# wangty537/raft_optical_flow

Measured on AMD Instinct MI355X. Metric: image-pairs/s at Sintel 436x1024, 32 iters; corr-lookup GB/s vs HBM peak, higher is better.
Workload: dtype fp32 (convs: f16x3 split MFMA, fp32 accumulate); 1 GPU; RAFT-full inference, 436x1024 padded to 440x1024, 1 pair(s)/GPU/step, iters=32, all-pairs corr, hipGraph; global_batch=1, parallelism=frame-pair sharding x1

## Files before the change

include/raft_hip.h:

```cpp
#ifndef RAFT_HIP_H_
#define RAFT_HIP_H_

#include <stddef.h>

#ifdef __cplusplus
extern "C" {
#endif

#define RAFT_HIP_ABI_VERSION 19

#define RAFT_E_INVALID (-1)
#define RAFT_E_ALIGN (-2)

typedef void* raft_stream_t;

int raft_hip_abi_version(void);
const char* raft_hip_arch(void);
const char* raft_hip_last_error(void);
const char* raft_hip_source_hash(void);
int raft_debug_launch_span(int enable);
int raft_debug_launch_span_read(unsigned long long* host, int n);
int raft_debug_fill_lds_nan(raft_stream_t stream);

size_t raft_corr_pyramid_floats(int B, int H, int W, int num_levels);
int raft_corr_build(const float* fmap1, const float* fmap2, int ld, int B, int H, int W, int C,
                    int num_levels, float sqrt_c, float* pyramid, raft_stream_t stream);
int raft_corr_build_prec(const float* fmap1, const float* fmap2, int ld, int B, int H, int W, int C,
                         int num_levels, float sqrt_c, int precision, float* pyramid, raft_stream_t stream);
size_t raft_corr_build_ws_bytes(int B, int H, int W, int C);
size_t raft_corr_build_ws_bytes_prec(int B, int H, int W, int C, int precision);
int raft_corr_build_ws(const float* fmap1, const float* fmap2, int ld, int B, int H, int W, int C,
                       int num_levels, float sqrt_c, int precision, float* pyramid, void* ws, size_t ws_bytes,
                       raft_stream_t stream);
int raft_corr_pyramid_level(const float* pyramid, int B, int H, int W, int num_levels, int level,
                            float* out, raft_stream_t stream);

int raft_corr_lookup(const float* pyramid, int B, int H, int W, int num_levels, int radius,
                     const float* coords, int coords_layout, float* out, int out_ld, int out_layout,
                     float* flow_out, int flow_ld, int* range_flag, raft_stream_t stream);
int raft_corr_lookup_convf1(const float* pyramid, int B, int H, int W, int num_levels, int radius,
                            const float* coords, int coords_layout, float* out, int out_ld, int out_layout,
                            float* flow_out, int flow_ld, int* range_flag, const float* f1_weight,
                            const float* f1_bias, int f1_n, int f1_k, int f1_precision, float* f1_out,
                            int f1_out_ld, int* f1_range_flag, raft_stream_t stream);
int raft_convf1_flow(const float* coords, int coords_layout, int B, int H, int W, const float* f1_weight,
                     const float* f1_bias, int f1_n, int f1_k, int f1_precision, float* f1_out, int f1_out_ld,
                     int* f1_range_flag, raft_stream_t stream);

int raft_corr_lookup_conv(const float* pyramid, int B, int H, int W, int num_levels, int radius,
                          const float* coords, float* flow_out, int flow_ld, int* range_flag, int precision,
                          const void* c1_weight, const float* c1_bias, int c1_n, float* c1_out, int c1_out_ld,
                          int* c1_range_flag, const void* f1_weight, const float* f1_bias, int f1_n, int f1_k,
                          float* f1_out, int f1_out_ld, int* f1_range_flag, raft_stream_t stream);
size_t raft_lookup_conv_weight_floats(int n, int k_pad);
int raft_lookup_conv_pack_weight(const void* split_weight, int n_pad, int k_pad, int n, void* out,
                                 raft_stream_t stream);
// ... 249 lines not shown
```

raft_optical_flow_amd/_lib.py:

```python
from __future__ import annotations

import ctypes
import os
import threading

_HERE = os.path.dirname(os.path.abspath(__file__))
LIB_PATH = os.environ.get("RAFT_HIP_LIB") or os.path.join(_HERE, "libraft_hip.so")

c_int = ctypes.c_int
c_float = ctypes.c_float
c_size_t = ctypes.c_size_t
c_long = ctypes.c_long
c_void_p = ctypes.c_void_p
c_char_p = ctypes.c_char_p
P = c_void_p

RAFT_CONV_VEC = 0
RAFT_CONV_GATHER = 1

PREC_FP32 = 0
PREC_F16X3 = 1
PREC_F16 = 2
PREC_BF16 = 3
PRECISIONS = {"fp32": PREC_FP32, "f16x3": PREC_F16X3, "f16": PREC_F16, "bf16": PREC_BF16}
# ... 99 lines not shown
    f = ConvForm()
    call("raft_conv2d_form", ctypes.byref(p), ctypes.byref(f))
    return f


def conv_pair_form(p0: ConvParams, p1: ConvParams):
    f = (ConvForm * 2)()
    one = c_int(0)
    call("raft_conv2d_pair_form", ctypes.byref(p0), ctypes.byref(p1), f, ctypes.byref(one))
    return f[0], f[1], bool(one.value)


_PROTOS = {
    "raft_hip_abi_version": (c_int, []),
    "raft_hip_arch": (c_char_p, []),
    "raft_hip_last_error": (c_char_p, []),
    "raft_hip_source_hash": (c_char_p, []),
    "raft_debug_fill_lds_nan": (c_int, [P]),
    "raft_corr_pyramid_floats": (c_size_t, [c_int, c_int, c_int, c_int]),
    "raft_corr_build": (c_int, [P, P, c_int, c_int, c_int, c_int, c_int, c_int, c_float, P, P]),
    "raft_corr_build_prec": (c_int, [P, P, c_int, c_int, c_int, c_int, c_int, c_int, c_float, c_int, P, P]),
    "raft_corr_build_ws_bytes": (c_size_t, [c_int, c_int, c_int, c_int]),
    "raft_corr_build_ws_bytes_prec": (c_size_t, [c_int, c_int, c_int, c_int, c_int]),
    "raft_corr_build_ws": (c_int, [P, P, c_int, c_int, c_int, c_int, c_int, c_int, c_float, c_int, P, P, c_size_t, P]),
    "raft_corr_pyramid_level": (c_int, [P, c_int, c_int, c_int, c_int, c_int, P, P]),
    "raft_corr_lookup": (c_int, [P, c_int, c_int, c_int, c_int, c_int, P, c_int, P, c_int, c_int, P, c_int, P, P]),
    "raft_corr_lookup_convf1": (c_int, [P, c_int, c_int, c_int, c_int, c_int, P, c_int, P, c_int, c_int, P, c_int, P,
                                        P, P, c_int, c_int, c_int, P, c_int, P, P]),
    "raft_convf1_flow": (c_int, [P, c_int, c_int, c_int, c_int, P, P, c_int, c_int, c_int, P, c_int, P, P]),
    "raft_corr_lookup_conv": (c_int, [P, c_int, c_int, c_int, c_int, c_int, P, P, c_int, P, c_int, P, P, c_int, P,
                                      c_int, P, P, P, c_int, c_int, P, c_int, P, P]),
    "raft_lookup_conv_weight_floats": (c_size_t, [c_int, c_int]),
    "raft_lookup_conv_pack_weight": (c_int, [P, c_int, c_int, c_int, P, P]),
    "raft_alt_corr_forward": (c_int, [P, P, P, P, c_int, c_int, c_int, c_int, c_int, c_int, c_int, c_int, c_float, P]),
    "raft_alt_corr_forward_prec": (c_int, [P, P, P, P, c_int, c_int, c_int, c_int, c_int, c_int, c_int, c_int, c_float,
                                           c_int, P]),
    "raft_alt_corr_lookup_levels_prec": (c_int, [P, P, P, P, c_int, P, c_int, P, c_int, c_int, c_int, c_int, c_int,
                                                 c_int, ctypes.c_float, P, c_int, P, c_int, P]),
    "raft_alt_corr_lookup_nhwc_prec": (c_int, [P, P, P, c_int, c_float, P, c_int, c_int, c_int, c_int, c_int, c_int,
                                               c_int, c_int, c_float, P, c_int, P, c_int, P]),
    "raft_alt_corr_lookup_levels": (c_int, [P, P, P, P, c_int, P, c_int, P, c_int, c_int, c_int, c_int, c_int, c_int,
                                            ctypes.c_float, P, c_int, P, P]),
    "raft_alt_corr_lookup_nhwc": (c_int, [P, P, P, c_int, c_float, P, c_int, c_int, c_int, c_int, c_int, c_int, c_int,
                                          c_int, c_float, P, c_int, P, P]),
    "raft_alt_corr_backward": (c_int, [P, P, P, P, P, P, P, c_int, c_int, c_int, c_int, c_int, c_int, c_int, c_int,
                                       P, c_size_t, P]),
# ... 134 lines not shown
```

raft_optical_flow_amd/csrc/corr_pyramid.hip:

```cpp
#include "lookup_common.hpp"

namespace raft {
namespace {



constexpr int CB_BM = 64, CB_BN = 64, CB_BK = 32, CB_LDSK = CB_BK + 4;

struct CorrBuildArgs {
  const float* f1;
  const float* f2;
  int ld, H, W, C, P;
  float sqrt_c;
  float* pyr;
  Level l0, l1;
  int has_l1;
  int nbx;
  int nt;
  int B, mt, ntl, gm, nfast, xcd;
};

template <bool X3>
__global__ __launch_bounds__(256) void corr_build_kernel(CorrBuildArgs a) {
  constexpr int STAGE = (CB_BM + CB_BN) * CB_LDSK;
// ... 290 lines not shown
        const int xx = tj * 4 + c;
        float v = 0.f;
        if (by * 4 + yy < a.l1.h && bx * 8 + xx < a.l1.w) {
          const float* t = T + row * CB2_TLD + (2 * yy) * 16 + 2 * xx;
          const float2 u0 = *reinterpret_cast<const float2*>(t), u1 = *reinterpret_cast<const float2*>(t + 16);
          v = (((u0.x + u0.y) + u1.x) + u1.y) / 4.0f;
        }
        v4[c] = v;
      }
      f32x4* dst = reinterpret_cast<f32x4*>(a.pyr + a.l1.off + ((long)b * a.P + p1) * a.l1.mapsz +
                                            ((long)by * a.l1.tw + tx1) * 16 + e);
      if (a.nt)
        __builtin_nontemporal_store(v4, dst);
      else
        *dst = v4;
    }
  }
}

constexpr int CB4_T = 256;
constexpr int CB4_ROW = 64;
constexpr int CB4_STAGE = 2 * CB4_T * CB4_ROW;
constexpr int CB4_NS = 4;

struct CB4Args {
  const char* s1;
  const char* s2;
  unsigned sbytes;
  int H, W, P, nh;
  float sqrt_c;
  float* pyr;
  Level l0, l1, l2;
  int nt;
  int qt, ttx, tt;
  long units;
  f32x4* sink;
};

__global__ __launch_bounds__(256) void corr_split4_kernel(const float* __restrict__ f, int ld, long npix, int C,
                                                          char* __restrict__ out) {
  const long i = (long)blockIdx.x * 256 + threadIdx.x;
  const int ng = C / 4;
  if (i >= npix * ng) return;
  const long px = i / ng;
  const int g = (int)(i - px * ng);
  const f32x4 v = *reinterpret_cast<const f32x4*>(f + px * ld + 4 * g);
  h4 hi, lo;
#pragma unroll
  for (int e = 0; e < 4; ++e) {
    const _Float16 h = (_Float16)v[e];
    hi[e] = h;
    lo[e] = (_Float16)(v[e] - (float)h);
  }
  char* r = out + px * (long)C * 4 + (g >> 2) * CB4_ROW + (g & 3) * 8;
  *reinterpret_cast<h4*>(r) = hi;
  *reinterpret_cast<h4*>(r + 32) = lo;
}

#ifdef CB4_STAMPS
__device__ unsigned long long g_cb4stamp[8 * 8 * 1024];
__device__ __forceinline__ unsigned long long cb4_clock() {
  unsigned long long t;
  __builtin_amdgcn_sched_barrier(0);
// ... 18 lines not shown
  constexpr int TQ = NW == 8 ? CB4_T : CB4_T / 2;
  constexpr int ROWS = CB4_T + TQ;
  constexpr int NS = NW == 8 ? CB4_NS : 3;
  constexpr int AHEAD = NS - 1;
  constexpr int STAGE = ROWS * CB4_ROW;
  constexpr int NDMA = ROWS / 16 / NW;
  constexpr int TDMA = 16 / NW;
#ifdef CB4_STAMPS
  unsigned long long cb4_t[6] = {}, cb4_prev = cb4_clock();
  const unsigned long long cb4_start = cb4_prev;
  int cb4_units = 0;
#endif
  constexpr int NSTORE = 8 * (4 + (L1 ? 1 : 0)) + (L2 ? 4 : 0);
  __shared__ __attribute__((aligned(1024))) char smem[NS * STAGE];
  const int lane = threadIdx.x & 63;
  const int w = __builtin_amdgcn_readfirstlane(threadIdx.x >> 6);
  const int wm = w & 3, wn = NW == 8 ? w >> 2 : 0;
  const int m = lane & 31, h = lane >> 5;
  const long grid = gridDim.x;
  const unsigned rowb = (unsigned)a.nh * CB4_ROW;
  const __amdgpu_buffer_rsrc_t rq = make_rsrc(a.s1, a.sbytes), rt = make_rsrc(a.s2, a.sbytes);
  struct Unit {
    int b, q0, ty0, tx0;
  };
  auto unit_at = [&](long u) {
    Unit t;
    const long per = (long)a.qt * a.tt;
    t.b = (int)(u / per);
    const long r = u - (long)t.b * per;
    const int qi = (int)(r / a.tt), ti = (int)(r - (long)qi * a.tt);
    t.q0 = qi * TQ;
    t.ty0 = (ti / a.ttx) * 16;
    t.tx0 = (ti % a.ttx) * 16;
    return t;
  };
  unsigned voff[NDMA];
  auto set_offsets = [&](const Unit& t) {
#pragma unroll
    for (int k = 0; k < NDMA; ++k) {
      const int row = 16 * (w + NW * k) + (lane >> 2);
      const unsigned lq = (unsigned)((lane & 3) ^ ((row >> 1) & 3));
      bool ok;
      long px;
      if (k < TDMA) {
        const int R = row, mm = R & 31, c = (R >> 5) & 1;
        const int h2 = t.ty0 + 4 * (R >> 6) + (mm >> 3), w2 = t.tx0 + 8 * c + 4 * ((mm >> 2) & 1) + (mm & 3);
        ok = h2 < a.H && w2 < a.W;
        px = (long)t.b * a.P + (long)h2 * a.W + w2;
      } else {
        const int p1 = t.q0 + row - CB4_T;
        ok = p1 < a.P;
        px = (long)t.b * a.P + p1;
      }
      voff[k] = ok ? (unsigned)px * rowb + lq * 16u : OFF_INVALID;
    }
  };
  const long total = a.units;
  long u_is = blockIdx.x;
  int s_is = 0;
  long g_is = 0;
  if (u_is >= total) return;
  set_offsets(unit_at(u_is));
  auto issue = [&]() {
    const bool live = u_is < total;
    char* st = smem + (g_is % NS) * STAGE;
#pragma unroll
    for (int k = 0; k < NDMA; ++k)
      dma16(k < TDMA ? rt : rq, st + (w + NW * k) * 1024, live ? voff[k] : OFF_INVALID, (unsigned)s_is * CB4_ROW);
    ++g_is;
    if (++s_is == a.nh) {
      s_is = 0;
      u_is += grid;
      if (u_is < total) set_offsets(unit_at(u_is));
    }
  };
#pragma unroll
  for (int k = 0; k < AHEAD; ++k) issue();
  const int arow0 = wm * 64 + m, brow0 = CB4_T + wn * 128 + m;
  f32x16 acc[2][4];
#pragma unroll
  for (int c = 0; c < 2; ++c)
#pragma unroll
    for (int j = 0; j < 4; ++j) acc[c][j] = f32x16{};
  long g = 0;
  int since = AHEAD;
  for (long u = blockIdx.x; u < total; u += grid) {
    for (int s = 0; s < a.nh; ++s, ++g, ++since) {
      CB4_ST(5);
      if (since <= AHEAD - 1)
        wait_vm<NDMA * (AHEAD - 1) + NSTORE>();
      else
        wait_vm<NDMA * (AHEAD - 1)>();
      CB4_ST(0);
      asm volatile("s_barrier" ::: "memory");
      CB4_ST(1);
      issue();
      CB4_ST(2);
      const char* st = smem + (g % NS) * STAGE;
      h8 ah[2], al[2], bh[4], bl[4];
#pragma unroll
      for (int c = 0; c < 2; ++c) {
        const int row = arow0 + 32 * c, sw = (row >> 1) & 3;
        ah[c] = *reinterpret_cast<const h8*>(st + row * CB4_ROW + ((h ^ sw) << 4));
        al[c] = *reinterpret_cast<const h8*>(st + row * CB4_ROW + (((2 + h) ^ sw) << 4));
      }
#pragma unroll
      for (int j = 0; j < 4; ++j) {
        const int row = brow0 + 32 * j, sw = (row >> 1) & 3;
        bh[j] = *reinterpret_cast<const h8*>(st + row * CB4_ROW + ((h ^ sw) << 4));
        bl[j] = *reinterpret_cast<const h8*>(st + row * CB4_ROW + (((2 + h) ^ sw) << 4));
      }
#pragma unroll
      for (int c = 0; c < 2; ++c)
#pragma unroll
        for (int j = 0; j < 4; ++j) acc[c][j] = __builtin_amdgcn_mfma_f32_32x32x16_f16(ah[c], bh[j], acc[c][j], 0, 0, 0);
#pragma unroll
      for (int c = 0; c < 2; ++c)
#pragma unroll
        for (int j = 0; j < 4; ++j) acc[c][j] = __builtin_amdgcn_mfma_f32_32x32x16_f16(al[c], bh[j], acc[c][j], 0, 0, 0);
#pragma unroll
      for (int c = 0; c < 2; ++c)
#pragma unroll
        for (int j = 0; j < 4; ++j) acc[c][j] = __builtin_amdgcn_mfma_f32_32x32x16_f16(ah[c], bl[j], acc[c][j], 0, 0, 0);
      CB4_ST(3);
    }
    const Unit t = unit_at(u);
    const int ty = t.ty0 / 4 + wm;
#pragma unroll
    for (int j = 0; j < 4; ++j) {
      const int p1 = t.q0 + wn * 128 + j * 32 + m;
      const bool qok = p1 < a.P;
      const long qb = (long)t.b * a.P + (qok ? p1 : 0);
      float l2v[2];
#pragma unroll
      for (int c = 0; c < 2; ++c) {
        const int tx = t.tx0 / 4 + 2 * c + h;
        float v[16];
#pragma unroll
        for (int r = 0; r < 16; ++r) v[r] = acc[c][j][r] / a.sqrt_c;
        {
          float rt[4][4];
#pragma unroll
          for (int e = 0; e < 4; ++e) {
#pragma unroll
            for (int i = 0; i < 4; ++i) rt[e][i] = v[4 * i + e];
            quad_transpose(rt[e]);
          }
          const int qr = lane & 3;
#pragma unroll
          for (int i = 0; i < 4; ++i) {
            const int pi = t.q0 + wn * 128 + j * 32 + (m & ~3) + i;
            const bool ok = pi < a.P && ty < a.l0.th && tx < a.l0.tw;
            f32x4* dst = ok ? reinterpret_cast<f32x4*>(a.pyr + a.l0.off + ((long)t.b * a.P + pi) * a.l0.mapsz +
                                                       ((long)ty * a.l0.tw + tx) * 16) + qr
                            : a.sink + 4 * lane + i;
            const f32x4 x = {rt[0][i], rt[1][i], rt[2][i], rt[3][i]};
            if (a.nt)
              __builtin_nontemporal_store(x, dst);
            else
              *dst = x;
          }
        }
        if constexpr (L1) {
          float pv[2][2];
#pragma unroll
          for (int ya = 0; ya < 2; ++ya)
#pragma unroll
            for (int xb = 0; xb < 2; ++xb) {
              const float s = ((v[8 * ya + 2 * xb] + v[8 * ya + 2 * xb + 1]) + v[8 * ya + 4 + 2 * xb]) + v[8 * ya + 4 + 2 * xb + 1];
              const bool in = 2 * ty + ya < a.l1.h && 2 * tx + xb < a.l1.w;
              pv[ya][xb] = in ? s / 4.0f : 0.f;
            }
          const float o0 = __shfl_xor(pv[1 - h][0], 32), o1 = __shfl_xor(pv[1 - h][1], 32);
          const f32x4 row4 = h == 0 ? f32x4{pv[0][0], pv[0][1], o0, o1} : f32x4{o0, o1, pv[1][0], pv[1][1]};
// ... 6 lines not shown
            __builtin_nontemporal_store(row4, dst);
          else
            *dst = row4;
          if constexpr (L2) {
            const bool in2 = ty < a.l2.h && tx < a.l2.w;
            l2v[c] = in2 ? (((pv[0][0] + pv[0][1]) + pv[1][0]) + pv[1][1]) / 4.0f : 0.f;
          }
        }
      }
      if constexpr (L2) {
        const float o0 = __shfl_xor(l2v[0], 32), o1 = __shfl_xor(l2v[1], 32);
        const int ty2 = t.ty0 >> 4, tx2 = t.tx0 >> 4;
        const bool ok = qok && h == 0 && ty2 < a.l2.th && tx2 < a.l2.tw;
        f32x4* dst = ok ? reinterpret_cast<f32x4*>(a.pyr + a.l2.off + qb * a.l2.mapsz + ((long)ty2 * a.l2.tw + tx2) * 16 +
                                                   wm * 4)
                        : a.sink + 4 * lane;
        const f32x4 row4 = {l2v[0], o0, l2v[1], o1};
        if (a.nt)
          __builtin_nontemporal_store(row4, dst);
        else
          *dst = row4;
      }
    }
#pragma unroll
    for (int c = 0; c < 2; ++c)
#pragma unroll
      for (int j = 0; j < 4; ++j) acc[c][j] = f32x16{};
    since = 0;
    CB4_ST(4);
#ifdef CB4_STAMPS
    ++cb4_units;
#endif
  }
  wait_vm<0>();
#ifdef CB4_STAMPS
  if (lane == 0 && blockIdx.x < 1024) {
    unsigned long long* gs = g_cb4stamp + ((long)blockIdx.x * 8 + w) * 8;
    for (int k = 0; k < 6; ++k) gs[k] = cb4_t[k];
    gs[6] = cb4_clock() - cb4_start;
    gs[7] = (unsigned long long)cb4_units;
  }
#endif
}

__global__ void pool2_tiled_kernel(const float* pyr, float* out_base, long n_maps, Level src,
                                   Level dst) {
  const long total = n_maps * dst.mapsz;
  for (long i = blockIdx.x * (long)blockDim.x + threadIdx.x; i < total; i += (long)gridDim.x * blockDim.x) {
    const long q = i / dst.mapsz;
    const int r = (int)(i - q * dst.mapsz);
    const int tile = r >> 4, e = r & 15;
    const int y = (tile / dst.tw) * 4 + (e >> 2), x = (tile % dst.tw) * 4 + (e & 3);
    float v = 0.f;
    if (y < dst.h && x < dst.w) {
      const float* m = pyr + src.off + q * src.mapsz;
// ... 495 lines not shown
#ifdef CB4_STAMPS
extern "C" int raft_debug_cb4stamps(unsigned long long* host, int n) {
  return (int)hipMemcpyFromSymbol(host, HIP_SYMBOL(g_cb4stamp), sizeof(unsigned long long) * (size_t)n);
}
#endif

extern "C" size_t raft_corr_build_ws_bytes(int B, int H, int W, int C) {
  if (B <= 0 || H <= 0 || W <= 0 || C <= 0) return 0;
  return 2 * (size_t)B * H * W * C * 4 + 4096;
}

namespace raft {
static bool corr_build4_shape(int B, int H, int W, int C, int precision) {
  if (env_off("RAFT_CORR_BUILD4")) return false;
  return precision == RAFT_PREC_F16X3 && C % 16 == 0 && C >= 64 && C <= 1024 && B > 0 && H > 0 && W > 0 &&
         (double)B * H * W * C * 4 < 2147483648.0;
}
}

extern "C" size_t raft_corr_build_ws_bytes_prec(int B, int H, int W, int C, int precision) {
  return raft::corr_build4_shape(B, H, W, C, precision) ? raft_corr_build_ws_bytes(B, H, W, C) : 0;
}

extern "C" int raft_corr_build_ws(const float* fmap1, const float* fmap2, int ld, int B, int H, int W, int C, int L,
                                  float sqrt_c, int precision, float* pyramid, void* ws, size_t ws_bytes,
                                  raft_stream_t stream) {
  using namespace raft;
  const long P = (long)H * W;
  const bool fits = corr_build4_shape(B, H, W, C, precision) && ld % 4 == 0 && ld >= C && ws != nullptr &&
                    (((uintptr_t)fmap1 | (uintptr_t)fmap2 | (uintptr_t)pyramid | (uintptr_t)ws) & 15) == 0;
  if (!fits) return raft_corr_build_prec(fmap1, fmap2, ld, B, H, W, C, L, sqrt_c, precision, pyramid, stream);
  RAFT_REQUIRE(fmap1 && fmap2 && pyramid, "raft_corr_build_ws: null pointer");
  RAFT_REQUIRE(B > 0 && H > 0 && W > 0 && L >= 1 && L <= LK_MAXL, "raft_corr_build_ws: bad sizes");
  RAFT_REQUIRE(ws_bytes >= raft_corr_build_ws_bytes(B, H, W, C), "raft_corr_build_ws: workspace too small "
               "(raft_corr_build_ws_bytes)");
  RAFT_REQUIRE((((uintptr_t)fmap1 | (uintptr_t)fmap2 | (uintptr_t)pyramid | (uintptr_t)ws) & 15) == 0,
               "raft_corr_build_ws: fmaps, pyramid and workspace must be 16-byte aligned");
  Level lv[LK_MAXL];
  RAFT_REQUIRE(pyramid_levels(B, H, W, L, lv), "raft_corr_build_ws: a pyramid level is empty (%dx%d, %d levels)", H,
               W, L);
  hipStream_t s = as_stream(stream);
  const size_t map_bytes = (size_t)B * P * C * 4;
  char* s1 = static_cast<char*>(ws);
  char* s2 = s1 + map_bytes;
  const long nq = (long)B * P * (C / 4);
  hipLaunchKernelGGL(corr_split4_kernel, dim3((unsigned)cdiv_l(nq, 256)), dim3(256), 0, s, fmap1, ld, (long)B * P, C, s1);
  hipLaunchKernelGGL(corr_split4_kernel, dim3((unsigned)cdiv_l(nq, 256)), dim3(256), 0, s, fmap2, ld, (long)B * P, C, s2);
  int rc = check_launch("raft_corr_build_ws(split)");
  if (rc) return rc;
  CB4Args a;
  a.s1 = s1;
  a.s2 = s2;
  a.sbytes = (unsigned)map_bytes;
  a.H = H;
  a.W = W;
  a.P = (int)P;
  a.nh = C / 16;
  a.sqrt_c = sqrt_c;
  a.pyr = pyramid;
  a.l0 = lv[0];
  a.l1 = lv[L > 1 ? 1 : 0];
  a.l2 = lv[L > 2 ? 2 : 0];
  static const bool l2_off = env_off("RAFT_CB4_L2");
  const bool l2 = !l2_off && L > 2;
  a.nt = corr_nt(B, P, lv[0]);
  const bool w4 = env_on("RAFT_CB4_W4");
  a.qt = (int)cdiv_l(P, w4 ? CB4_T / 2 : CB4_T);
  a.ttx = cdiv(W, 16);
  a.tt = cdiv(H, 16) * a.ttx;
  a.units = (long)B * a.qt * a.tt;
  a.sink = reinterpret_cast<f32x4*>(s2 + map_bytes);
  const long wgs = (w4 ? 2L : 1L) * device_cus();
  const dim3 grid((unsigned)(a.units < wgs ? a.units : wgs));
  if (w4) {
    if (l2)
      hipLaunchKernelGGL((corr_build4_kernel<true, true, 4>), grid, dim3(256), 0, s, a);
    else if (L > 1)
      hipLaunchKernelGGL((corr_build4_kernel<true, false, 4>), grid, dim3(256), 0, s, a);
    else
      hipLaunchKernelGGL((corr_build4_kernel<false, false, 4>), grid, dim3(256), 0, s, a);
  } else if (l2) {
    hipLaunchKernelGGL((corr_build4_kernel<true, true>), grid, dim3(512), 0, s, a);
  } else if (L > 1) {
    hipLaunchKernelGGL(corr_build4_kernel<true>, grid, dim3(512), 0, s, a);
  } else {
    hipLaunchKernelGGL(corr_build4_kernel<false>, grid, dim3(512), 0, s, a);
  }
  rc = check_launch("raft_corr_build_ws");
  return rc ? rc : pool_levels(pyramid, B, P, lv, l2 ? 3 : 2, L, s, "raft_corr_build_ws(pool)");
}

extern "C" int raft_corr_pyramid_level(const float* pyramid, int B, int H, int W, int L, int level, float* out,
                                       raft_stream_t stream) {
  RAFT_REQUIRE(pyramid && out && B > 0 && H > 0 && W > 0 && L >= 1 && L <= LK_MAXL && level >= 0 && level < L,
               "raft_corr_pyramid_level: bad arguments");
  Level lv[LK_MAXL];
// ... 181 lines not shown
```

raft_optical_flow_amd/csrc/misc.hip:

```cpp
#include "common.hpp"

namespace raft {

char* last_error_buf() {
  static thread_local char buf[512] = {0};
  return buf;
}

namespace {

#define GRID_STRIDE(i, total) \
  for (long i = blockIdx.x * (long)blockDim.x + threadIdx.x; i < (total); i += (long)gridDim.x * blockDim.x)

__global__ void prep_images_kernel(const float* img1, const float* img2, float* out, int B, int H, int W) {
  const long HW = (long)H * W;
  const long total = 2L * B * HW * 3;
  GRID_STRIDE(i, total) {
    const int c = i % 3;
    const long pix = i / 3;
    const int bb = (int)(pix / HW);
    const long yx = pix - (long)bb * HW;
    const float* src = bb < B ? img1 + ((long)bb * 3 + c) * HW : img2 + ((long)(bb - B) * 3 + c) * HW;
    out[i] = 2.0f * (src[yx] / 255.0f) - 1.0f;
  }
// ... 224 lines not shown
  const double md = S / n;
  double var = SS / n - md * md;
  if (var < 0) var = 0;
  const double shift = x[(long)b * HW * ld + c];
  stats[2 * i] = (float)(shift + md);
  stats[2 * i + 1] = (float)(1.0 / sqrt(var + (double)eps));
}

__global__ void instnorm_apply_kernel(const float* x, int ld, const float* stats, const float* resid, int rld,
                                      const float* rstats, int mode, float* out, int old, int B, int HW, int C) {
  const long total = (long)B * HW * C;
  GRID_STRIDE(i, total) {
    const int c = i % C;
    const long pix = i / C;
    const int b = (int)(pix / HW);
    const float* st = stats + 2 * ((long)b * C + c);
    float v = (x[pix * ld + c] - st[0]) * st[1];
    if (mode >= 1) v = fmaxf(v, 0.f);
    if (resid) {
      float r = resid[pix * rld + c];
      if (rstats) {
        const float* rs = rstats + 2 * ((long)b * C + c);
        r = (r - rs[0]) * rs[1];
      }
      v = r + v;
      if (mode == 2) v = fmaxf(v, 0.f);
    }
    out[pix * old + c] = v;
  }
}

__global__ __launch_bounds__(256) void instnorm_apply4_kernel(const float* x, int ld, const float* stats,
                                                              const float* resid, int rld, const float* rstats, int mode,
                                                              float* out, int old, int HW, int nq, unsigned total) {
  for (unsigned i = blockIdx.x * 256u + threadIdx.x; i < total; i += gridDim.x * 256u) {
    const unsigned pix = i / (unsigned)nq, q = i - pix * (unsigned)nq;
    const unsigned b = pix / (unsigned)HW;
    const unsigned si = (b * (unsigned)nq + q) * 8u;
    const f32x4 s0 = *reinterpret_cast<const f32x4*>(stats + si), s1 = *reinterpret_cast<const f32x4*>(stats + si + 4);
    const f32x4 xv = *reinterpret_cast<const f32x4*>(x + (size_t)pix * ld + 4 * q);
    f32x4 v = {(xv[0] - s0[0]) * s0[1], (xv[1] - s0[2]) * s0[3], (xv[2] - s1[0]) * s1[1], (xv[3] - s1[2]) * s1[3]};
    if (mode >= 1) {
#pragma unroll
      for (int e = 0; e < 4; ++e) v[e] = fmaxf(v[e], 0.f);
    }
    if (resid) {
      f32x4 r = *reinterpret_cast<const f32x4*>(resid + (size_t)pix * rld + 4 * q);
      if (rstats) {
        const f32x4 r0 = *reinterpret_cast<const f32x4*>(rstats + si), r1 = *reinterpret_cast<const f32x4*>(rstats + si + 4);
        r = f32x4{(r[0] - r0[0]) * r0[1], (r[1] - r0[2]) * r0[3], (r[2] - r1[0]) * r1[1], (r[3] - r1[2]) * r1[3]};
      }
      v = r + v;
      if (mode == 2) {
#pragma unroll
        for (int e = 0; e < 4; ++e) v[e] = fmaxf(v[e], 0.f);
      }
    }
    *reinterpret_cast<f32x4*>(out + (size_t)pix * old + 4 * q) = v;
  }
}

__device__ __forceinline__ void chan_merge(double& n, double& mean, double& m2, double nb, double meanb, double m2b) {
  if (nb <= 0.0) return;
  const double nn = n + nb;
  const double d = meanb - mean;
  mean += d * (nb / nn);
  m2 += m2b + d * d * (n * nb / nn);
  n = nn;
}

__global__ __launch_bounds__(256) void instnorm_merge_kernel(const float* part, int slots, int C, int ld, float eps,
                                                             float* stats) {
  __shared__ double red[3][256];
  const int c = blockIdx.x, b = blockIdx.y, t = threadIdx.x;
  double n = 0.0, mean = 0.0, m2 = 0.0;
  constexpr int PF = 8;
// ... 404 lines not shown
extern "C" size_t raft_instnorm_merge_counters(int B, int C) {
  if (B <= 0 || C <= 0) return 0;
  return (size_t)B * cdiv(C, 64);
}

extern "C" int raft_instnorm_merge_fused(const float* part, int slots_per_image, int B, int C, int stats_ld, float eps,
                                         void* ws, int* counters, float* stats, raft_stream_t stream) {
  RAFT_REQUIRE(part && ws && counters && stats && slots_per_image > 0 && B > 0 && C > 0 && stats_ld >= C && B < 65536,
               "raft_instnorm_merge_fused: bad arguments");
  RAFT_REQUIRE(aligned16(part) && ((uintptr_t)ws & 7) == 0 && ((uintptr_t)counters & 3) == 0,
               "raft_instnorm_merge_fused: part 16-B, ws 8-B, counters 4-B aligned");
  const int G = cdiv(slots_per_image, MERGE_SPG);
  RAFT_REQUIRE(G < 65536, "raft_instnorm_merge_fused: too many slots");
  hipLaunchKernelGGL(instnorm_merge_fused_kernel, dim3(cdiv(C, 64), B, G), dim3(64 * MERGE2_WAVES), 0, as_stream(stream), part,
                     slots_per_image, C, stats_ld, reinterpret_cast<double*>(ws), G, eps, stats, counters);
  return check_launch("raft_instnorm_merge_fused");
}

extern "C" int raft_instnorm_apply(const float* x, int ld, const float* stats, const float* resid, int resid_ld,
                                   const float* resid_stats, int relu_mode, float* out, int out_ld, int B, int HW,
                                   int C, raft_stream_t stream) {
  RAFT_REQUIRE(x && stats && out && B > 0 && HW > 0 && C > 0 && ld >= C && out_ld >= C,
               "raft_instnorm_apply: bad arguments");
  RAFT_REQUIRE(relu_mode >= 0 && relu_mode <= 2, "raft_instnorm_apply: bad relu_mode");
  RAFT_REQUIRE(!resid || resid_ld >= C, "raft_instnorm_apply: bad resid_ld");
  const long n = (long)B * HW * C;
  const bool vec = C % 4 == 0 && ld % 4 == 0 && out_ld % 4 == 0 && aligned16(x) && aligned16(out) &&
                   aligned16(stats) && (!resid || (resid_ld % 4 == 0 && aligned16(resid))) &&
                   (!resid_stats || aligned16(resid_stats)) && n / 4 < (1L << 31);
  if (vec)
    hipLaunchKernelGGL(instnorm_apply4_kernel, dim3(grid_for(n / 4)), dim3(256), 0, as_stream(stream), x, ld, stats,
                       resid, resid_ld, resid_stats, relu_mode, out, out_ld, HW, C / 4, (unsigned)(n / 4));
  else
    hipLaunchKernelGGL(instnorm_apply_kernel, dim3(grid_for(n)), dim3(256), 0, as_stream(stream), x, ld, stats, resid,
                       resid_ld, resid_stats, relu_mode, out, out_ld, B, HW, C);
  return check_launch("raft_instnorm_apply");
}

extern "C" int raft_groupnorm_stats(const float* x, int ld, int B, int HW, int C, int G, float eps, float* stats,
                                    raft_stream_t stream) {
  RAFT_REQUIRE(x && stats && B > 0 && HW > 0 && C > 0 && G > 0 && C % G == 0 && ld >= C && B < 65536 && G < 65536,
               "raft_groupnorm_stats: bad arguments (C %% G == 0 required)");
  hipLaunchKernelGGL(groupnorm_stats_kernel, dim3(G, B), dim3(256), 0, as_stream(stream), x, ld, HW, C, G, eps, stats);
  return check_launch("raft_groupnorm_stats");
}

extern "C" int raft_norm_apply_affine(const float* x, int ld, const float* stats, const float* gamma, const float* beta,
// ... 27 lines not shown
```

raft_optical_flow_amd/engine.py:

```python
from __future__ import annotations

import ctypes
import os

import torch

from . import _lib
from . import kernels as K
from .kernels import Launch, PackedConv, Rows, conv_launch, conv_params, pack_conv, fold_bn, set_precision



def _conv_bn(conv, bn, device, **kw):
    if bn is None:
        return pack_conv(conv.weight, conv.bias, conv.stride, conv.padding, device=device, **kw)
    w, b = fold_bn(conv.weight, conv.bias, bn)
    return pack_conv(w, b, conv.stride, conv.padding, device=device, **kw)


def check_norm(norm, block=False):
    if norm not in ("instance", "batch", "none") and not (block and norm == "group"):
        raise NotImplementedError(f"norm_fn={norm!r} is not on the RAFT inference path")


# ... 160 lines not shown


def _in_apply(L, A: Arena, x: Rows, st, n_img, hw, mode, resid: Rows | None = None, rst=None) -> Rows:
    out = Rows(A.rows(n_img * hw, x.c))
    L.append(Launch("raft_instnorm_apply", x.ptr, x.ld, st.data_ptr(), resid.ptr if resid else None,
                    resid.ld if resid else 0, rst.data_ptr() if rst is not None else None, mode,
                    out.ptr, out.ld, n_img, hw, x.c))
    return out


_GUARD = {"flag": None}


def _conv(L, pc: PackedConv, src: Rows, n_img, h, w, out: Rows, side=False, **kw):
    kw.setdefault("range_flag", _GUARD["flag"])
    L.append(conv_launch(conv_params(pc, src, n_img, h, w, out, **kw), side=side))


def plan_encoder_trunk(L, A: Arena, pe: PackedEncoder, x: Rows, n_img, h, w):
    ho, wo = K.conv_out_hw(pe.stem, h, w)
    if pe.norm == "instance":
        t = Rows(A.rows(n_img * ho * wo, pe.stem.n))
        st = _conv_in(L, A, pe.stem, x, n_img, h, w, t)
        x = _in_apply(L, A, t, st, n_img, ho * wo, 1)
    else:
        t = Rows(A.rows(n_img * ho * wo, pe.stem.n))
        _conv(L, pe.stem, x, n_img, h, w, t, epilogue=_lib.EPI_RELU)
        x = t
    h, w = ho, wo
    for d in pe.blocks:
        if pe.small:
            x, h, w = _plan_bottleneck(L, A, pe, d, x, n_img, h, w)
        else:
            x, h, w = _plan_residual(L, A, pe, d, x, n_img, h, w)
    return x, h, w


def _gn_stats(L, A: Arena, x: Rows, n_img, hw, gn):
    st = A.flat(2 * n_img * x.c)
    L.append(Launch("raft_groupnorm_stats", x.ptr, x.ld, n_img, hw, x.c, gn[0], gn[3], st.data_ptr()))
    return st


def _gn_apply(L, A: Arena, x: Rows, st, gn, n_img, hw, mode, resid: Rows | None = None, rst=None, rgn=None) -> Rows:
    out = Rows(A.rows(n_img * hw, x.c))
    p = lambda t: t.data_ptr() if t is not None else None
# ... 27 lines not shown
def _plan_bottleneck_group(L, A, d, x: Rows, n, h, w):
    c1, c2, c3, ds = d["conv1"], d["conv2"], d["conv3"], d["ds"]
    ho, wo = K.conv_out_hw(c2, h, w)
    t1 = Rows(A.rows(n * h * w, c1.n))
    _conv(L, c1, x, n, h, w, t1)
    y1 = _gn_apply(L, A, t1, _gn_stats(L, A, t1, n, h * w, d["n1"]), d["n1"], n, h * w, 1)
    hw = ho * wo
    t2 = Rows(A.rows(n * hw, c2.n))
    _conv(L, c2, y1, n, h, w, t2)
    y2 = _gn_apply(L, A, t2, _gn_stats(L, A, t2, n, hw, d["n2"]), d["n2"], n, hw, 1)
    t3 = Rows(A.rows(n * hw, c3.n))
    _conv(L, c3, y2, n, ho, wo, t3)
    st3 = _gn_stats(L, A, t3, n, hw, d["n3"])
    if ds is not None:
        t4 = Rows(A.rows(n * hw, ds.n))
        _conv(L, ds, x, n, h, w, t4)
        out = _gn_apply(L, A, t3, st3, d["n3"], n, hw, 2, resid=t4, rst=_gn_stats(L, A, t4, n, hw, d["nds"]),
                        rgn=d["nds"])
    else:
        out = _gn_apply(L, A, t3, st3, d["n3"], n, hw, 2, resid=x)
    return out, ho, wo


def _plan_residual(L, A, pe, d, x: Rows, n, h, w):
    if pe.norm == "group":
        return _plan_residual_group(L, A, d, x, n, h, w)
    c1, c2, ds = d["conv1"], d["conv2"], d["ds"]
    ho, wo = K.conv_out_hw(c1, h, w)
    npx = n * ho * wo
    if pe.norm == "instance":
        t1 = Rows(A.rows(npx, c1.n))
        st1 = _conv_in(L, A, c1, x, n, h, w, t1)
        t2 = Rows(A.rows(npx, c2.n))
        if _norm_in_loader(c2, t1, n, ho, wo):
            st2 = _conv_in(L, A, c2, t1, n, ho, wo, t2, src_norm=st1)
        else:
            y1 = _in_apply(L, A, t1, st1, n, ho * wo, 1)
            st2 = _conv_in(L, A, c2, y1, n, ho, wo, t2)
        if ds is not None:
            t3 = Rows(A.rows(npx, ds.n))
            out = _in_apply(L, A, t2, st2, n, ho * wo, 2, resid=t3, rst=_conv_in(L, A, ds, x, n, h, w, t3))
        else:
            out = _in_apply(L, A, t2, st2, n, ho * wo, 2, resid=x)
        return out, ho, wo
    y1 = Rows(A.rows(npx, c1.n))
    _conv(L, c1, x, n, h, w, y1, epilogue=_lib.EPI_RELU)
    if ds is not None:
        xs = Rows(A.rows(npx, ds.n))
        _conv(L, ds, x, n, h, w, xs)
    else:
        xs = x
    out = Rows(A.rows(npx, c2.n))
    _conv(L, c2, y1, n, ho, wo, out, epilogue=_lib.EPI_RESID_RELU, aux0=xs)
    return out, ho, wo


def _plan_bottleneck(L, A, pe, d, x: Rows, n, h, w):
    if pe.norm == "group":
        return _plan_bottleneck_group(L, A, d, x, n, h, w)
    c1, c2, c3, ds = d["conv1"], d["conv2"], d["conv3"], d["ds"]
    ho, wo = K.conv_out_hw(c2, h, w)
    if pe.norm == "instance":
        t1 = Rows(A.rows(n * h * w, c1.n))
        st1 = _conv_in(L, A, c1, x, n, h, w, t1)
# ... 663 lines not shown
```

Measured before the change: 142.3 image-pairs/s.

## Balance corr-build tail by splitting units, merge split4 launches, fuse stem instnorm

The corr-build kernel's work units are rescheduled: when the last round of units would leave most CUs idle, the tail units are split into 2 or 4 narrower query sub-tiles (NJ columns), each specialised at compile time, with a cost model picking the split. The two fmap split4 conversion launches are merged into one 2-D grid launch. Separately, an opt-in path (RAFT_IN_NORM=2) folds the stem instance-norm into the first residual block's conv loader and residual apply with a new relu mode 3. Splitting adds a per-item fixed overhead and more kernel variants, which raises register/code-size risk.

Result: no change. 141.8 image-pairs/s (-0.3%).

```diff
diff --git a/include/raft_hip.h b/include/raft_hip.h
--- a/include/raft_hip.h
+++ b/include/raft_hip.h
@@ -32,6 +32,7 @@
 int raft_corr_build_ws(const float* fmap1, const float* fmap2, int ld, int B, int H, int W, int C,
                        int num_levels, float sqrt_c, int precision, float* pyramid, void* ws, size_t ws_bytes,
                        raft_stream_t stream);
+int raft_corr_build_units(int B, int H, int W, int waves, int cus, long long* out);
 int raft_corr_pyramid_level(const float* pyramid, int B, int H, int W, int num_levels, int level,
                             float* out, raft_stream_t stream);
 
diff --git a/raft_optical_flow_amd/_lib.py b/raft_optical_flow_amd/_lib.py
--- a/raft_optical_flow_amd/_lib.py
+++ b/raft_optical_flow_amd/_lib.py
@@ -145,6 +145,7 @@
     "raft_corr_build_prec": (c_int, [P, P, c_int, c_int, c_int, c_int, c_int, c_int, c_float, c_int, P, P]),
     "raft_corr_build_ws_bytes": (c_size_t, [c_int, c_int, c_int, c_int]),
     "raft_corr_build_ws_bytes_prec": (c_size_t, [c_int, c_int, c_int, c_int, c_int]),
+    "raft_corr_build_units": (c_int, [c_int, c_int, c_int, c_int, c_int, P]),
     "raft_corr_build_ws": (c_int, [P, P, c_int, c_int, c_int, c_int, c_int, c_int, c_float, c_int, P, P, c_size_t, P]),
     "raft_corr_pyramid_level": (c_int, [P, c_int, c_int, c_int, c_int, c_int, P, P]),
     "raft_corr_lookup": (c_int, [P, c_int, c_int, c_int, c_int, c_int, P, c_int, P, c_int, c_int, P, c_int, P, P]),
diff --git a/raft_optical_flow_amd/csrc/corr_pyramid.hip b/raft_optical_flow_amd/csrc/corr_pyramid.hip
--- a/raft_optical_flow_amd/csrc/corr_pyramid.hip
+++ b/raft_optical_flow_amd/csrc/corr_pyramid.hip
@@ -336,6 +336,10 @@
 constexpr int CB4_ROW = 64;
 constexpr int CB4_STAGE = 2 * CB4_T * CB4_ROW;
 constexpr int CB4_NS = 4;
+template <int N>
+struct IntC {
+  static constexpr int value = N;
+};
 
 struct CB4Args {
   const char* s1;
@@ -348,11 +352,16 @@
   int nt;
   int qt, ttx, tt;
   long units;
+  long full, items;
+  int split;
   f32x4* sink;
 };
 
-__global__ __launch_bounds__(256) void corr_split4_kernel(const float* __restrict__ f, int ld, long npix, int C,
-                                                          char* __restrict__ out) {
+__global__ __launch_bounds__(256) void corr_split4_kernel(const float* __restrict__ fa, const float* __restrict__ fb,
+                                                          int ld, long npix, int C, char* __restrict__ outa,
+                                                          char* __restrict__ outb) {
+  const float* __restrict__ f = blockIdx.y ? fb : fa;
+  char* __restrict__ out = blockIdx.y ? outb : outa;
   const long i = (long)blockIdx.x * 256 + threadIdx.x;
   const int ng = C / 4;
   if (i >= npix * ng) return;
@@ -417,14 +426,24 @@
   const __amdgpu_buffer_rsrc_t rq = make_rsrc(a.s1, a.sbytes), rt = make_rsrc(a.s2, a.sbytes);
   struct Unit {
     int b, q0, ty0, tx0;
+    int nj;
   };
-  auto unit_at = [&](long u) {
+  auto unit_at = [&](long v) {
     Unit t;
+    long u = v;
+    int part = 0;
+    t.nj = 4;
+    if (v >= a.full) {
+      const long k = v - a.full;
+      u = a.full + k / a.split;
+      part = (int)(k % a.split);
+      t.nj = 4 / a.split;
+    }
     const long per = (long)a.qt * a.tt;
     t.b = (int)(u / per);
     const long r = u - (long)t.b * per;
     const int qi = (int)(r / a.tt), ti = (int)(r - (long)qi * a.tt);
-    t.q0 = qi * TQ;
+    t.q0 = qi * TQ + part * (TQ / a.split);
     t.ty0 = (ti / a.ttx) * 16;
     t.tx0 = (ti % a.ttx) * 16;
     return t;
@@ -443,14 +462,15 @@
         ok = h2 < a.H && w2 < a.W;
         px = (long)t.b * a.P + (long)h2 * a.W + w2;
       } else {
-        const int p1 = t.q0 + row - CB4_T;
-        ok = p1 < a.P;
+        const int r = row - CB4_T;
+        const int p1 = t.q0 + (r >> 7) * 32 * t.nj + (r & 127);
+        ok = ((r >> 5) & 3) < t.nj && p1 < a.P;
         px = (long)t.b * a.P + p1;
       }
       voff[k] = ok ? (unsigned)px * rowb + lq * 16u : OFF_INVALID;
     }
   };
-  const long total = a.units;
+  const long total = a.items;
   long u_is = blockIdx.x;
   int s_is = 0;
   long g_is = 0;
@@ -472,18 +492,20 @@
 #pragma unroll
   for (int k = 0; k < AHEAD; ++k) issue();
   const int arow0 = wm * 64 + m, brow0 = CB4_T + wn * 128 + m;
-  f32x16 acc[2][4];
-#pragma unroll
-  for (int c = 0; c < 2; ++c)
-#pragma unroll
-    for (int j = 0; j < 4; ++j) acc[c][j] = f32x16{};
   long g = 0;
   int since = AHEAD;
-  for (long u = blockIdx.x; u < total; u += grid) {
+  auto run_item = [&](auto njc, long u) {
+    constexpr int NJ = decltype(njc)::value;
+    constexpr int NST = NSTORE * NJ / 4;
+    f32x16 acc[2][NJ];
+#pragma unroll
+    for (int c = 0; c < 2; ++c)
+#pragma unroll
+      for (int j = 0; j < NJ; ++j) acc[c][j] = f32x16{};
     for (int s = 0; s < a.nh; ++s, ++g, ++since) {
       CB4_ST(5);
       if (since <= AHEAD - 1)
-        wait_vm<NDMA * (AHEAD - 1) + NSTORE>();
+        wait_vm<NDMA * (AHEAD - 1) + NST>();
       else
         wait_vm<NDMA * (AHEAD - 1)>();
       CB4_ST(0);
@@ -492,7 +514,7 @@
       issue();
       CB4_ST(2);
       const char* st = smem + (g % NS) * STAGE;
-      h8 ah[2], al[2], bh[4], bl[4];
+      h8 ah[2], al[2], bh[NJ], bl[NJ];
 #pragma unroll
       for (int c = 0; c < 2; ++c) {
         const int row = arow0 + 32 * c, sw = (row >> 1) & 3;
@@ -500,7 +522,7 @@
         al[c] = *reinterpret_cast<const h8*>(st + row * CB4_ROW + (((2 + h) ^ sw) << 4));
       }
 #pragma unroll
-      for (int j = 0; j < 4; ++j) {
+      for (int j = 0; j < NJ; ++j) {
         const int row = brow0 + 32 * j, sw = (row >> 1) & 3;
         bh[j] = *reinterpret_cast<const h8*>(st + row * CB4_ROW + ((h ^ sw) << 4));
         bl[j] = *reinterpret_cast<const h8*>(st + row * CB4_ROW + (((2 + h) ^ sw) << 4));
@@ -508,22 +530,22 @@
 #pragma unroll
       for (int c = 0; c < 2; ++c)
 #pragma unroll
-        for (int j = 0; j < 4; ++j) acc[c][j] = __builtin_amdgcn_mfma_f32_32x32x16_f16(ah[c], bh[j], acc[c][j], 0, 0, 0);
+        for (int j = 0; j < NJ; ++j) acc[c][j] = __builtin_amdgcn_mfma_f32_32x32x16_f16(ah[c], bh[j], acc[c][j], 0, 0, 0);
 #pragma unroll
       for (int c = 0; c < 2; ++c)
 #pragma unroll
-        for (int j = 0; j < 4; ++j) acc[c][j] = __builtin_amdgcn_mfma_f32_32x32x16_f16(al[c], bh[j], acc[c][j], 0, 0, 0);
+        for (int j = 0; j < NJ; ++j) acc[c][j] = __builtin_amdgcn_mfma_f32_32x32x16_f16(al[c], bh[j], acc[c][j], 0, 0, 0);
 #pragma unroll
       for (int c = 0; c < 2; ++c)
 #pragma unroll
-        for (int j = 0; j < 4; ++j) acc[c][j] = __builtin_amdgcn_mfma_f32_32x32x16_f16(ah[c], bl[j], acc[c][j], 0, 0, 0);
+        for (int j = 0; j < NJ; ++j) acc[c][j] = __builtin_amdgcn_mfma_f32_32x32x16_f16(ah[c], bl[j], acc[c][j], 0, 0, 0);
       CB4_ST(3);
     }
     const Unit t = unit_at(u);
     const int ty = t.ty0 / 4 + wm;
 #pragma unroll
-    for (int j = 0; j < 4; ++j) {
-      const int p1 = t.q0 + wn * 128 + j * 32 + m;
+    for (int j = 0; j < NJ; ++j) {
+      const int p1 = t.q0 + wn * (32 * NJ) + j * 32 + m;
       const bool qok = p1 < a.P;
       const long qb = (long)t.b * a.P + (qok ? p1 : 0);
       float l2v[2];
@@ -544,7 +566,7 @@
           const int qr = lane & 3;
 #pragma unroll
           for (int i = 0; i < 4; ++i) {
-            const int pi = t.q0 + wn * 128 + j * 32 + (m & ~3) + i;
+            const int pi = t.q0 + wn * (32 * NJ) + j * 32 + (m & ~3) + i;
             const bool ok = pi < a.P && ty < a.l0.th && tx < a.l0.tw;
             f32x4* dst = ok ? reinterpret_cast<f32x4*>(a.pyr + a.l0.off + ((long)t.b * a.P + pi) * a.l0.mapsz +
                                                        ((long)ty * a.l0.tw + tx) * 16) + qr
@@ -597,15 +619,23 @@
           *dst = row4;
       }
     }
-#pragma unroll
-    for (int c = 0; c < 2; ++c)
-#pragma unroll
-      for (int j = 0; j < 4; ++j) acc[c][j] = f32x16{};
     since = 0;
     CB4_ST(4);
 #ifdef CB4_STAMPS
     ++cb4_units;
 #endif
+  };
+  for (long u = blockIdx.x; u < total; u += grid) {
+    if constexpr (NW == 8) {
+      if (u < a.full)
+        run_item(IntC<4>{}, u);
+      else if (a.split == 2)
+        run_item(IntC<2>{}, u);
+      else
+        run_item(IntC<1>{}, u);
+    } else {
+      run_item(IntC<4>{}, u);
+    }
   }
   wait_vm<0>();
 #ifdef CB4_STAMPS
@@ -1147,6 +1177,60 @@
   return raft::corr_build4_shape(B, H, W, C, precision) ? raft_corr_build_ws_bytes(B, H, W, C) : 0;
 }
 
+namespace raft {
+constexpr double CB4_PART_FIXED = 0.16;
+constexpr double CB4_MIN_GAIN = 0.03;
+struct CB4Sched {
+  int waves, tq;
+  int qt, ttx, tt;
+  long units, grid;
+  long full, items;
+  int split;
+  double cost, cost_plain;
+};
+static CB4Sched cb4_schedule(int B, int H, int W, int waves, long cus, bool balance) {
+  CB4Sched s;
+  const long P = (long)H * W;
+  s.waves = waves;
+  s.tq = waves == 4 ? CB4_T / 2 : CB4_T;
+  s.qt = (int)cdiv_l(P, s.tq);
+  s.ttx = cdiv(W, 16);
+  s.tt = cdiv(H, 16) * s.ttx;
+  s.units = (long)B * s.qt * s.tt;
+  const long wgs = (waves == 4 ? 2L : 1L) * cus;
+  s.grid = s.units < wgs ? s.units : wgs;
+  const long rounds = s.units / wgs, tail = s.units % wgs;
+  s.cost_plain = (double)(rounds + (tail ? 1 : 0));
+  s.full = s.units;
+  s.split = 1;
+  s.cost = s.cost_plain;
+  if (balance && waves == 8 && rounds >= 1 && tail > 0) {
+    for (int split = 2; split <= 4; split *= 2) {
+      const double c = (double)rounds + (double)cdiv_l(tail * split, wgs) * (1.0 + CB4_PART_FIXED * (split - 1)) / split;
+      if (c < s.cost && c <= (1.0 - CB4_MIN_GAIN) * s.cost_plain) {
+        s.cost = c;
+        s.split = split;
+        s.full = s.units - tail;
+      }
+    }
+  }
+  s.items = s.full + (s.units - s.full) * s.split;
+  return s;
+}
+}
+
+extern "C" int raft_corr_build_units(int B, int H, int W, int waves, int cus, long long* out) {
+  using namespace raft;
+  RAFT_REQUIRE(out && B > 0 && H > 0 && W > 0 && (waves == 0 || waves == 4 || waves == 8) && cus >= 0,
+               "raft_corr_build_units: bad arguments");
+  if (waves == 0) waves = env_on("RAFT_CB4_W4") ? 4 : 8;
+  const CB4Sched s = cb4_schedule(B, H, W, waves, cus > 0 ? (long)cus : device_cus(), !env_off("RAFT_CB4_BALANCE"));
+  const long long v[12] = {s.waves, s.tq,   s.qt,    s.ttx,   s.tt, s.units, s.grid, s.full, s.split,
+                           s.items, (long long)(s.cost * 1000.0 + 0.5), (long long)(s.cost_plain * 1000.0 + 0.5)};
+  for (int i = 0; i < 12; ++i) out[i] = v[i];
+  return 0;
+}
+
 extern "C" int raft_corr_build_ws(const float* fmap1, const float* fmap2, int ld, int B, int H, int W, int C, int L,
                                   float sqrt_c, int precision, float* pyramid, void* ws, size_t ws_bytes,
                                   raft_stream_t stream) {
@@ -1169,8 +1253,8 @@
   char* s1 = static_cast<char*>(ws);
   char* s2 = s1 + map_bytes;
   const long nq = (long)B * P * (C / 4);
-  hipLaunchKernelGGL(corr_split4_kernel, dim3((unsigned)cdiv_l(nq, 256)), dim3(256), 0, s, fmap1, ld, (long)B * P, C, s1);
-  hipLaunchKernelGGL(corr_split4_kernel, dim3((unsigned)cdiv_l(nq, 256)), dim3(256), 0, s, fmap2, ld, (long)B * P, C, s2);
+  hipLaunchKernelGGL(corr_split4_kernel, dim3((unsigned)cdiv_l(nq, 256), 2), dim3(256), 0, s, fmap1, fmap2, ld,
+                     (long)B * P, C, s1, s2);
   int rc = check_launch("raft_corr_build_ws(split)");
   if (rc) return rc;
   CB4Args a;
@@ -1190,13 +1274,16 @@
   const bool l2 = !l2_off && L > 2;
   a.nt = corr_nt(B, P, lv[0]);
   const bool w4 = env_on("RAFT_CB4_W4");
-  a.qt = (int)cdiv_l(P, w4 ? CB4_T / 2 : CB4_T);
-  a.ttx = cdiv(W, 16);
-  a.tt = cdiv(H, 16) * a.ttx;
-  a.units = (long)B * a.qt * a.tt;
+  const CB4Sched sc = cb4_schedule(B, H, W, w4 ? 4 : 8, device_cus(), !env_off("RAFT_CB4_BALANCE"));
+  a.qt = sc.qt;
+  a.ttx = sc.ttx;
+  a.tt = sc.tt;
+  a.units = sc.units;
+  a.full = sc.full;
+  a.items = sc.items;
+  a.split = sc.split;
   a.sink = reinterpret_cast<f32x4*>(s2 + map_bytes);
-  const long wgs = (w4 ? 2L : 1L) * device_cus();
-  const dim3 grid((unsigned)(a.units < wgs ? a.units : wgs));
+  const dim3 grid((unsigned)sc.grid);
   if (w4) {
     if (l2)
       hipLaunchKernelGGL((corr_build4_kernel<true, true, 4>), grid, dim3(256), 0, s, a);
diff --git a/raft_optical_flow_amd/csrc/misc.hip b/raft_optical_flow_amd/csrc/misc.hip
--- a/raft_optical_flow_amd/csrc/misc.hip
+++ b/raft_optical_flow_amd/csrc/misc.hip
@@ -270,9 +270,10 @@
       if (rstats) {
         const float* rs = rstats + 2 * ((long)b * C + c);
         r = (r - rs[0]) * rs[1];
+        if (mode == 3) r = fmaxf(r, 0.f);
       }
       v = r + v;
-      if (mode == 2) v = fmaxf(v, 0.f);
+      if (mode >= 2) v = fmaxf(v, 0.f);
     }
     out[pix * old + c] = v;
   }
@@ -297,9 +298,13 @@
       if (rstats) {
         const f32x4 r0 = *reinterpret_cast<const f32x4*>(rstats + si), r1 = *reinterpret_cast<const f32x4*>(rstats + si + 4);
         r = f32x4{(r[0] - r0[0]) * r0[1], (r[1] - r0[2]) * r0[3], (r[2] - r1[0]) * r1[1], (r[3] - r1[2]) * r1[3]};
+        if (mode == 3) {
+#pragma unroll
+          for (int e = 0; e < 4; ++e) r[e] = fmaxf(r[e], 0.f);
+        }
       }
       v = r + v;
-      if (mode == 2) {
+      if (mode >= 2) {
 #pragma unroll
         for (int e = 0; e < 4; ++e) v[e] = fmaxf(v[e], 0.f);
       }
@@ -750,7 +755,9 @@
                                    int C, raft_stream_t stream) {
   RAFT_REQUIRE(x && stats && out && B > 0 && HW > 0 && C > 0 && ld >= C && out_ld >= C,
                "raft_instnorm_apply: bad arguments");
-  RAFT_REQUIRE(relu_mode >= 0 && relu_mode <= 2, "raft_instnorm_apply: bad relu_mode");
+  RAFT_REQUIRE(relu_mode >= 0 && relu_mode <= 3, "raft_instnorm_apply: bad relu_mode");
+  RAFT_REQUIRE(relu_mode != 3 || (resid && resid_stats), "raft_instnorm_apply: relu_mode 3 normalises the residual "
+               "(resid and resid_stats)");
   RAFT_REQUIRE(!resid || resid_ld >= C, "raft_instnorm_apply: bad resid_ld");
   const long n = (long)B * HW * C;
   const bool vec = C % 4 == 0 && ld % 4 == 0 && out_ld % 4 == 0 && aligned16(x) && aligned16(out) &&
diff --git a/raft_optical_flow_amd/engine.py b/raft_optical_flow_amd/engine.py
--- a/raft_optical_flow_amd/engine.py
+++ b/raft_optical_flow_amd/engine.py
@@ -206,6 +206,12 @@
     if pe.norm == "instance":
         t = Rows(A.rows(n_img * ho * wo, pe.stem.n))
         st = _conv_in(L, A, pe.stem, x, n_img, h, w, t)
+        b0 = pe.blocks[0] if pe.blocks and not pe.small and os.environ.get("RAFT_IN_NORM", "1") == "2" else None
+        if b0 is not None and b0["ds"] is None and _norm_in_loader(b0["conv1"], t, n_img, ho, wo):
+            x, h, w = _plan_residual(L, A, pe, b0, t, n_img, ho, wo, x_norm=st)
+            for d in pe.blocks[1:]:
+                x, h, w = _plan_residual(L, A, pe, d, x, n_img, h, w)
+            return x, h, w
         x = _in_apply(L, A, t, st, n_img, ho * wo, 1)
     else:
         t = Rows(A.rows(n_img * ho * wo, pe.stem.n))
@@ -279,15 +285,16 @@
     return out, ho, wo
 
 
-def _plan_residual(L, A, pe, d, x: Rows, n, h, w):
+def _plan_residual(L, A, pe, d, x: Rows, n, h, w, x_norm=None):
     if pe.norm == "group":
         return _plan_residual_group(L, A, d, x, n, h, w)
     c1, c2, ds = d["conv1"], d["conv2"], d["ds"]
     ho, wo = K.conv_out_hw(c1, h, w)
     npx = n * ho * wo
+    assert x_norm is None or (pe.norm == "instance" and ds is None)
     if pe.norm == "instance":
         t1 = Rows(A.rows(npx, c1.n))
-        st1 = _conv_in(L, A, c1, x, n, h, w, t1)
+        st1 = _conv_in(L, A, c1, x, n, h, w, t1, src_norm=x_norm)
         t2 = Rows(A.rows(npx, c2.n))
         if _norm_in_loader(c2, t1, n, ho, wo):
             st2 = _conv_in(L, A, c2, t1, n, ho, wo, t2, src_norm=st1)
@@ -297,6 +304,8 @@
         if ds is not None:
             t3 = Rows(A.rows(npx, ds.n))
             out = _in_apply(L, A, t2, st2, n, ho * wo, 2, resid=t3, rst=_conv_in(L, A, ds, x, n, h, w, t3))
+        elif x_norm is not None:
+            out = _in_apply(L, A, t2, st2, n, ho * wo, 3, resid=x, rst=x_norm)
         else:
             out = _in_apply(L, A, t2, st2, n, ho * wo, 2, resid=x)
         return out, ho, wo
```
